# ocrickard/piper-swift

Hardware: AMD Instinct MI355X
Metric: audio-sec/wall-sec (RTF^-1) with ms/utterance, Piper VITS en_GB-medium geometry, scale-bench factor (higher is better)
Workload: dtype f32; 1 GPU; medium factor=8: 112 ids, 336 frames, 86016 samples (3.901 s audio) per utterance, 1 utterance per step per GPU; factor=8, phoneme_count=112, frames=336, samples=86016, parallelism=utterance-replicas x1 (one-shot RCCL weight broadcast)

## Files before the change

### piper-swift_amd/csrc/conv_win.h

```cpp
#pragma once
#include "common.h"

namespace ph {

struct ConvWinArgs {
  const float* x = nullptr;
  const float* x2 = nullptr;
  const float* x3 = nullptr;
  const float* w4 = nullptr;
  const float* bias = nullptr;
  const float* res = nullptr;
  const float* mrf_a = nullptr;
  const float* mrf_b = nullptr;
  float* y = nullptr;
  float pro_alpha = 1.0f;
  float out_alpha = 1.0f;
  int N = 1, Cin = 0, Cout = 0, K = 1, dil = 1, padL = 0;
  int Lin = 0;
  int Lout = 0;
  int y_len = 0;
  int ct_stride = 0, ct_pad = 0;
  const int* len_ptr = nullptr;
  int len_mul = 1;
};

size_t packed_conv_win_floats(int Cout, int Cin, int K);
size_t packed_convt_win_floats(int Cin, int Cout, int K, int stride);
int pack_conv_weights_win(hipStream_t s, const float* w, int Cout, int Cin, int K, float* packed);
int pack_convt_weights_win(hipStream_t s, const float* w, int Cin, int Cout, int K, int stride, int pad, float* packed);

bool conv_win_eligible(int Cout, int Cin, int K, int dil, int padL, int Lin, int Lout);
bool convt_win_eligible(int Cin, int Cout, int K, int stride, int pad, int Lin);

int launch_conv_win(piper_hip_ctx* ctx, hipStream_t s, const ConvWinArgs& a);
constexpr int kWinMulti = 3;
int launch_conv_win_multi(piper_hip_ctx* ctx, hipStream_t s, const ConvWinArgs* convs, int count);

size_t packed_conv_pipe_floats(int Cout, int Cin, int K);
size_t packed_convt_pipe_floats(int Cin, int Cout, int K, int stride);
int pack_conv_weights_pipe(hipStream_t s, const float* w, int Cout, int Cin, int K, float* packed);
int pack_convt_weights_pipe(hipStream_t s, const float* w, int Cin, int Cout, int K, int stride, int pad, float* packed);
bool conv_pipe_eligible(int Cout, int Cin, int K, int dil, int padL, int Lin, int Lout);
bool convt_pipe_eligible(int Cin, int Cout, int K, int stride, int pad, int Lin);
int launch_conv_pipe_multi(piper_hip_ctx* ctx, hipStream_t s, const ConvWinArgs* convs, int count);

struct RbPairArgs {
  const float* x = nullptr;
  float* y = nullptr;
  const float *wa4 = nullptr, *ba = nullptr, *wb4 = nullptr, *bb = nullptr;
  int Ka = 1, dila = 1, Kb = 1, dilb = 1;
  int res_a = 1, res_b_x = 0;
  float alpha = 0.1f;
  int N = 1, C = 0, L = 0;
  const int* len_ptr = nullptr;
  int len_mul = 1;
};
bool rb_pair_eligible(int C, int Ka, int dila, int Kb, int dilb, int L);
int launch_rb_pair_multi(piper_hip_ctx* ctx, hipStream_t s, const RbPairArgs* pairs, int count);

}
```

### piper-swift_amd/csrc/rb_pair.hip

```cpp
#include <algorithm>
#include <type_traits>

#include "conv_win.h"

namespace ph {
namespace {

typedef float f32x16 __attribute__((ext_vector_type(16)));

constexpr int kRA = 8;
constexpr int kStepPad = 16;
constexpr int kWN = 4, kNTW = 2, kT1 = kWN * kNTW;
constexpr int kColsA = 32 * kT1;
__host__ __device__ constexpr int halo_of(int pb) { return pb <= 16 ? 16 : 48; }
constexpr int kMaxReachB = 48;
constexpr int kStageU = 10;

struct RbPairMulti {
  RbPairArgs c[kWinMulti];
};

#ifdef PH_PAIR_TRACE
__device__ unsigned long long* ph_pair_trace_buf;
#define PH_STAMP(k) do { if (lane == 0 && round < 4 && ph_pair_trace_buf && blockIdx.x < 512) ph_pair_trace_buf[(((size_t)blockIdx.x * (MT * kWN) + wave) * 4 + round) * 8 + (k)] = __builtin_amdgcn_s_memtime(); } while (0)
#else
#define PH_STAMP(k) do { } while (0)
#endif

__device__ __forceinline__ float lrelu_max(float v, float alpha) { return fmaxf(v, v * alpha); }

__device__ __forceinline__ float bload(__amdgpu_buffer_rsrc_t r, int voff, int soff) {
  return __builtin_bit_cast(float, __builtin_amdgcn_raw_buffer_load_b32(r, voff, soff, 0));
}
__device__ __forceinline__ void bstore(__amdgpu_buffer_rsrc_t r, float v, int voff, int soff) {
  __builtin_amdgcn_raw_buffer_store_b32(__builtin_bit_cast(int, v), r, voff, soff, 0);
}

struct PairSched {
  int ntx[kWinMulti];
  int cnt[kWinMulti];
  int total, batch, order;
};

template <int MT>
__global__ __launch_bounds__(MT * kWN * 64, 2) void rb_pair_kernel(const RbPairMulti multi, const PairSched sch, const int Wx, const int W1,
                                                               const unsigned inv_w4) {
  extern __shared__ __attribute__((aligned(16))) float lds[];
  constexpr int BT = MT * kWN * 64;
  const int lane = threadIdx.x & 63;
  const int wave = __builtin_amdgcn_readfirstlane((int)(threadIdx.x >> 6));
  const int wm = wave % MT, wn = wave / MT;
  const int r = lane & 31, h = lane >> 5;
  constexpr int C = 32 * MT, C2 = C >> 1;
  float* xs = lds;
  float* x1s = lds + C * Wx + 4;
  float* biasS = x1s + C * W1;
  for (int i = threadIdx.x; i < kWinMulti * 2 * C; i += BT) {
    const int z = i / (2 * C), rem = i - z * 2 * C;
    const RbPairArgs& p = multi.c[(sch.order >> (4 * z)) & 15];
    biasS[i] = rem < C ? p.ba[rem] : p.bb[rem - C];
  }
  const int rowlane = wm * 32 + 4 * h;
  const unsigned lane16 = (unsigned)lane * 16u;
  const int G = (int)gridDim.x, bid = (int)blockIdx.x;

  struct Tile {
    const float *x, *wa4, *wb4;
    float* y;
    int bias_off;
    int Ka, dila, Kb, dilb, res_a, res_b_x, L, Lv, pa, pb, halo, c0, ga, shift, Sa, Spa, Sb, Spb, ntb;
    float alpha;
  };
  auto tile_index = [&](int round) {
    const int idx = round * G + ((round & 1) ? G - 1 - bid : bid);
    return idx < sch.total ? idx : -1;
  };
  auto setup = [&](int idx) {
    int z = 0, rem = idx;
    if (rem >= sch.cnt[0]) { rem -= sch.cnt[0]; z = 1; }
    if (z == 1 && rem >= sch.cnt[1]) { rem -= sch.cnt[1]; z = 2; }
    const RbPairArgs& p = multi.c[(sch.order >> (4 * z)) & 15];
    const int ntx = sch.ntx[z];
    const int n = __builtin_amdgcn_readfirstlane(rem / ntx);
    const int bx = rem - n * ntx;
    Tile t;
    t.x = p.x + (int64_t)n * C * p.L;
    t.y = p.y + (int64_t)n * C * p.L;
    t.wa4 = p.wa4; t.wb4 = p.wb4; t.bias_off = z * 2 * C;
    t.Ka = p.Ka; t.dila = p.dila; t.Kb = p.Kb; t.dilb = p.dilb; t.res_a = p.res_a; t.res_b_x = p.res_b_x; t.L = p.L; t.alpha = p.alpha;
    t.Lv = p.len_ptr ? min(p.len_ptr[n] * p.len_mul, p.L) : p.L;
    t.pa = (p.Ka - 1) * p.dila / 2; t.pb = (p.Kb - 1) * p.dilb / 2;
    t.halo = halo_of(t.pb);
    const int ncb = kColsA - 2 * t.halo;
    t.c0 = bx * ncb;
    const int g0 = t.c0 - t.halo - t.pa;
    t.ga = g0 & ~3;
    t.shift = g0 - t.ga;
    t.Sa = p.Ka * C2; t.Spa = (t.Sa + kStepPad - 1) / kStepPad * kStepPad;
    t.Sb = p.Kb * C2; t.Spb = (t.Sb + kStepPad - 1) / kStepPad * kStepPad;
    t.ntb = min(max((ncb >> 5) - wn * kNTW, 0), kNTW);
    return t;
  };

  float4 a[kRA];
  const char* wa = nullptr;
  auto load_a = [&](int slot, int ahead) { a[slot] = *(const float4*)(wa + ahead * 1024 + lane16); };
  auto ring_start = [&](const float* w4, int Sp) {
    wa = (const char*)w4 + (int64_t)wm * Sp * 256;
#pragma unroll
    for (int d = 0; d < kRA - 1; d++) load_a(d, d);
  };

  float4 pre[kStageU];
  const int W4 = Wx >> 2, total4 = C * W4;
  auto stage_issue = [&](const Tile& t, const int tx) {
#pragma unroll
    for (int u = 0; u < kStageU; u++) {
      const int ic = min(tx + u * BT, total4 - 1);
      const int row = (int)__umulhi((unsigned)ic, inv_w4);
      const int pos = t.ga + 4 * (ic - row * W4);
      pre[u] = *(const float4*)(t.x + (int64_t)row * t.L + ((pos >= 0 && pos < t.L) ? pos : 0));
    }
  };
  auto stage_commit = [&](const Tile& t, const int tx) {
#pragma unroll
    for (int u = 0; u < kStageU; u++) {
      const int i = tx + u * BT;
      const int ic = min(i, total4 - 1);
      const int row = (int)__umulhi((unsigned)ic, inv_w4);
      const int i4 = ic - row * W4;
      const int pos = t.ga + 4 * i4;
      const int nv = (pos >= 0 && pos < t.L) ? t.Lv - pos : 0;
      float4 v = pre[u];
      v.x = nv > 0 ? lrelu_max(v.x, t.alpha) : 0.0f; v.y = nv > 1 ? lrelu_max(v.y, t.alpha) : 0.0f;
      v.z = nv > 2 ? lrelu_max(v.z, t.alpha) : 0.0f; v.w = nv > 3 ? lrelu_max(v.w, t.alpha) : 0.0f;
      *(float4*)(xs + (i < total4 ? row * Wx + 4 * i4 : C * Wx)) = v;
    }
  };

  f32x16 acc[kNTW];
  auto run_conv = [&](auto nt_tag, const float* img, const int Wrow, const int S, const int Sp, const int dil, const int col0, const int bias_off) {
    constexpr int NT = decltype(nt_tag)::value;
#pragma unroll
    for (int g4 = 0; g4 < 4; g4++) {
      const float4 bv = *(const float4*)(biasS + bias_off + rowlane + 8 * g4);
#pragma unroll
      for (int j = 0; j < kNTW; j++) { acc[j][4 * g4] = bv.x; acc[j][4 * g4 + 1] = bv.y; acc[j][4 * g4 + 2] = bv.z; acc[j][4 * g4 + 3] = bv.w; }
    }
    const int lbase = h * Wrow + col0 + r;
    int sidx = 0, c_n = 0, left = S - 1;
    const int wrap_delta = dil - 2 * Wrow * (C2 - 1);
    float b[2][NT][4];
    auto read_b4 = [&](int slot) {
#pragma unroll
      for (int e = 0; e < 4; e++) {
#pragma unroll
        for (int j = 0; j < NT; j++) b[slot][j][e] = img[lbase + sidx + 32 * j];
        c_n++;
        const bool wrap = c_n == C2;
        c_n = wrap ? 0 : c_n;
        const int delta = wrap ? wrap_delta : 2 * Wrow;
        sidx += left > 0 ? delta : 0;
        left--;
      }
    };
    auto group = [&](int u) {
      load_a((u + kRA - 1) % kRA, kRA - 1 + u);
      read_b4((u + 1) & 1);
      __builtin_amdgcn_sched_barrier(0);
      const float av[4] = {a[u].x, a[u].y, a[u].z, a[u].w};
#pragma unroll
      for (int e = 0; e < 4; e++)
#pragma unroll
        for (int j = 0; j < NT; j++) acc[j] = __builtin_amdgcn_mfma_f32_32x32x2f32(av[e], b[u & 1][j][e], acc[j], 0, 0, 0);
    };
    read_b4(0);
    const int Gr = Sp >> 2, full = Gr / kRA;
    if (full > 0) {
#pragma unroll
      for (int u = 0; u < kRA; u++) group(u);
      wa += kRA * 1024;
    }
    for (int g = 1; g < full; g++) {
#pragma unroll
      for (int u = 0; u < kRA; u++) group(u);
      wa += kRA * 1024;
    }
    const int rem = Gr - full * kRA;
#pragma unroll
    for (int u = 0; u < kRA - 1; u++)
      if (u < rem) group(u);
  };

  Tile cur = setup(tile_index(0));
  ring_start(cur.wa4, cur.Spa);
  stage_issue(cur, (int)threadIdx.x);
  stage_commit(cur, (int)threadIdx.x);
  __syncthreads();

  for (int round = 0;; round++) {
    const int nidx = tile_index(round + 1);
    const bool has_next = nidx >= 0;
    const Tile nxt = has_next ? setup(nidx) : cur;
    int tx = (int)threadIdx.x, rl = rowlane, rr = r;
    asm volatile("" : "+v"(tx), "+v"(rl), "+v"(rr));
    float resx[kNTW][16];
    auto load_res = [&](int gres0) {
      const __amdgpu_buffer_rsrc_t rx = __builtin_amdgcn_make_buffer_rsrc((void*)cur.x, 0, C * cur.L * 4, 0x00020000);
#pragma unroll
      for (int j = 0; j < kNTW; j++) {
        const int g = gres0 + (wn * kNTW + j) * 32 + rr;
        const int voff = (g >= 0 && g < cur.L) ? (rl * cur.L + g) * 4 : -4;
#pragma unroll
        for (int q = 0; q < 16; q++) resx[j][q] = bload(rx, voff, ((q & 3) + 8 * (q >> 2)) * cur.L * 4);
      }
    };

    PH_STAMP(0);
    __builtin_amdgcn_s_waitcnt(0x0F70);
    PH_STAMP(1);
    if (has_next) stage_issue(nxt, tx);

    const bool live = cur.c0 < cur.Lv;
    if (live) run_conv(std::integral_constant<int, kNTW>{}, xs, Wx, cur.Sa, cur.Spa, cur.dila, cur.shift + wn * kNTW * 32, cur.bias_off);
    PH_STAMP(2);
    if (live) ring_start(cur.wb4, cur.Spb);
    if (live && cur.res_a) load_res(cur.c0 - cur.halo);
    __syncthreads();
    PH_STAMP(3);

    if (live) {
#pragma unroll
      for (int j = 0; j < kNTW; j++) {
        const int colw = (wn * kNTW + j) * 32 + rr;
        const int g = cur.c0 - cur.halo + colw;
        const bool in = g >= 0 && g < cur.Lv;
#pragma unroll
        for (int q = 0; q < 16; q++) {
          const int rq = (q & 3) + 8 * (q >> 2);
          const int o = (rl + rq) * W1 + colw;
          float v = acc[j][q];
          if (cur.res_a) v += resx[j][q];
          v = in ? v : 0.0f;
          x1s[o] = lrelu_max(v, cur.alpha);
          if (!cur.res_b_x) xs[o] = v;
        }
      }
    }
    __syncthreads();

    PH_STAMP(4);
    if (live && cur.ntb > 0) {
      const int col0b = cur.halo - cur.pb + wn * kNTW * 32;
      __builtin_amdgcn_s_waitcnt(0x0F70);
      if (cur.ntb == 2) run_conv(std::integral_constant<int, 2>{}, x1s, W1, cur.Sb, cur.Spb, cur.dilb, col0b, cur.bias_off + C);
      else run_conv(std::integral_constant<int, 1>{}, x1s, W1, cur.Sb, cur.Spb, cur.dilb, col0b, cur.bias_off + C);
    }
    PH_STAMP(5);
    if (has_next) ring_start(nxt.wa4, nxt.Spa);
    if (live && cur.res_b_x && cur.ntb > 0) load_res(cur.c0);
    if (live && cur.ntb > 0) {
      const __amdgpu_buffer_rsrc_t ry = __builtin_amdgcn_make_buffer_rsrc((void*)cur.y, 0, C * cur.L * 4, 0x00020000);
#pragma unroll
      for (int j = 0; j < kNTW; j++) {
        if (j >= cur.ntb) break;
        const int colo = (wn * kNTW + j) * 32 + rr;
        const int g = cur.c0 + colo;
        const int voff = g < cur.L ? (rl * cur.L + g) * 4 : -4;
#pragma unroll
        for (int q = 0; q < 16; q++) {
          const int rq = (q & 3) + 8 * (q >> 2);
          float v = acc[j][q];
          v += cur.res_b_x ? resx[j][q] : xs[(rl + rq) * W1 + cur.halo + colo];
          bstore(ry, v, voff, rq * cur.L * 4);
        }
      }
    }
    PH_STAMP(6);
    if (!has_next) break;
    __syncthreads();
    stage_commit(nxt, tx);
    __syncthreads();
    PH_STAMP(7);
    cur = nxt;
  }
}

struct PairGeom {
  int Wx, W1;
  size_t lds;
};

PairGeom pair_geom(int C, int pa_max, int pb_max) {
  auto pad = [](int w, bool odd32) {
    w = (w + 3) & ~3;
    if (odd32) while ((w & 63) != 32) w += 4;
    return w;
  };
  PairGeom g;
  for (int pass = 0; pass < 2; pass++) {
    g.Wx = pad(kColsA + 2 * pa_max + 3, pass == 0);
    g.W1 = pad(kColsA, pass == 0);
    (void)pb_max;
    g.lds = ((size_t)C * g.Wx + 4 + (size_t)C * g.W1 + (size_t)kWinMulti * 2 * C) * sizeof(float);
    if (g.lds <= 160 * 1024 && (C * g.Wx) / 4 <= kStageU * (C / 32) * kWN * 64) break;
  }
  return g;
}

template <int MT>
void launch_pair_inst(piper_hip_ctx* ctx, hipStream_t s, const RbPairMulti& m, const PairSched& sch, const PairGeom& g) {
  static bool raised[kMaxDevices] = {};
  if (g.lds > 64 * 1024 && lds_optin_needed(raised))
    (void)hipFuncSetAttribute((const void*)rb_pair_kernel<MT>, hipFuncAttributeMaxDynamicSharedMemorySize, 160 * 1024);
  const unsigned inv = (unsigned)(0x100000000ull / (unsigned)(g.Wx >> 2)) + 1u;
  const int per_cu = std::max(1, std::min(2, (int)((size_t)160 * 1024 / g.lds)));
  const int grid = std::min(sch.total, per_cu * ctx->num_cus);
  hipLaunchKernelGGL((rb_pair_kernel<MT>), dim3(grid), dim3(MT * kWN * 64), g.lds, s, m, sch, g.Wx, g.W1, inv);
}

}

#ifdef PH_PAIR_TRACE
void rb_pair_set_trace(unsigned long long* buf) { (void)hipMemcpyToSymbol(HIP_SYMBOL(ph_pair_trace_buf), &buf, sizeof buf); }
#endif

bool rb_pair_eligible(int C, int Ka, int dila, int Kb, int dilb, int L) {
  if (C != 32 && C != 64) return false;
  if (Ka < 1 || Kb < 1 || !(Ka & 1) || !(Kb & 1) || dila < 1 || dilb < 1) return false;
  if (L < 4 || (L & 3)) return false;
  const int pa = (Ka - 1) * dila / 2, pb = (Kb - 1) * dilb / 2;
  if (pb > kMaxReachB) return false;
  if ((int64_t)C * (kColsA + 2 * pa + 70) >= (1 << 20)) return false;
  const PairGeom g = pair_geom(C, pa, pb);
  return g.lds <= 160 * 1024 && (C * g.Wx) / 4 <= kStageU * (C / 32) * kWN * 64;
}

int launch_rb_pair_multi(piper_hip_ctx* ctx, hipStream_t s, const RbPairArgs* pairs, int count) {
  if (count < 1 || count > kWinMulti) PH_FAIL(PIPER_HIP_ERR_ARG, "rb_pair: %d pairs in one launch (1..%d)", count, kWinMulti);
  const RbPairArgs& a = pairs[0];
  if (a.N <= 0 || a.L <= 0) return PIPER_HIP_OK;
  int pa_max = 0, pb_max = 0;
  int idx[kWinMulti] = {0, 1, 2};
  for (int i = 0; i < count; i++) {
    const RbPairArgs& b = pairs[i];
    if (b.N != a.N || b.C != a.C || b.L != a.L) PH_FAIL(PIPER_HIP_ERR_SHAPE, "rb_pair: pairs of one launch must share N, C and L");
    if (!rb_pair_eligible(b.C, b.Ka, b.dila, b.Kb, b.dilb, b.L)) PH_FAIL(PIPER_HIP_ERR_UNSUPPORTED, "rb_pair: geometry not covered (C=%d K=%d,%d d=%d,%d L=%d)", b.C, b.Ka, b.Kb, b.dila, b.dilb, b.L);
    if (!(b.alpha > 0.0f && b.alpha < 1.0f)) PH_FAIL(PIPER_HIP_ERR_UNSUPPORTED, "rb_pair: LeakyReLU slope %g outside (0,1)", (double)b.alpha);
    if (!b.x || !b.y || !b.wa4 || !b.wb4 || !b.ba || !b.bb) PH_FAIL(PIPER_HIP_ERR_ARG, "rb_pair: null operand");
    pa_max = std::max(pa_max, (b.Ka - 1) * b.dila / 2);
    pb_max = std::max(pb_max, (b.Kb - 1) * b.dilb / 2);
  }
  const PairGeom g = pair_geom(a.C, pa_max, pb_max);
  if (g.lds > 160 * 1024 || (a.C * g.Wx) / 4 > kStageU * (a.C / 32) * kWN * 64)
    PH_FAIL(PIPER_HIP_ERR_UNSUPPORTED, "rb_pair: window of %zu bytes (row %d) exceeds LDS / the staging registers", g.lds, g.Wx);
  std::sort(idx, idx + count, [&](int l, int r2) { return pairs[l].Ka + pairs[l].Kb > pairs[r2].Ka + pairs[r2].Kb; });
  PairSched sch = {};
  sch.batch = a.N;
  for (int i = 0; i < count; i++) {
    const RbPairArgs& b = pairs[idx[i]];
    sch.order |= idx[i] << (4 * i);
    sch.ntx[i] = (int)ceil_div(a.L, kColsA - 2 * halo_of((b.Kb - 1) * b.dilb / 2));
    sch.cnt[i] = sch.ntx[i] * a.N;
    sch.total += sch.cnt[i];
  }
  for (int i = count; i < kWinMulti; i++) { sch.ntx[i] = 1; sch.cnt[i] = 0; }
  RbPairMulti m;
  for (int i = 0; i < kWinMulti; i++) m.c[i] = pairs[i < count ? i : 0];
  if (a.C == 32) launch_pair_inst<1>(ctx, s, m, sch, g);
  else launch_pair_inst<2>(ctx, s, m, sch, g);
  hipError_t e = hipGetLastError();
  if (e != hipSuccess) PH_FAIL(PIPER_HIP_ERR_LAUNCH, "rb_pair launch failed: %s", hipGetErrorString(e));
  return PIPER_HIP_OK;
}

}
namespace ph { namespace { PH_WARM(rb_pair, (rb_pair_kernel<1>)); } }
```

Before: 5373 audio-sec/wall-sec.

## Add streaming rb_pair kernel that walks columns with a rolling halo window

```diff
diff --git a/piper-swift_amd/csrc/conv_win.h b/piper-swift_amd/csrc/conv_win.h
--- a/piper-swift_amd/csrc/conv_win.h
+++ b/piper-swift_amd/csrc/conv_win.h
@@ -57,5 +57,6 @@
 };
 bool rb_pair_eligible(int C, int Ka, int dila, int Kb, int dilb, int L);
 int launch_rb_pair_multi(piper_hip_ctx* ctx, hipStream_t s, const RbPairArgs* pairs, int count);
+bool launch_rb_pair_stream(piper_hip_ctx* ctx, hipStream_t s, const RbPairArgs* pairs, int count);
 
 }
diff --git a/piper-swift_amd/csrc/rb_pair.hip b/piper-swift_amd/csrc/rb_pair.hip
--- a/piper-swift_amd/csrc/rb_pair.hip
+++ b/piper-swift_amd/csrc/rb_pair.hip
@@ -1,40 +1,20 @@
 #include <algorithm>
 #include <type_traits>
 
-#include "conv_win.h"
+#include "rb_pair_common.h"
 
 namespace ph {
 namespace {
 
-typedef float f32x16 __attribute__((ext_vector_type(16)));
-
-constexpr int kRA = 8;
-constexpr int kStepPad = 16;
-constexpr int kWN = 4, kNTW = 2, kT1 = kWN * kNTW;
 constexpr int kColsA = 32 * kT1;
 __host__ __device__ constexpr int halo_of(int pb) { return pb <= 16 ? 16 : 48; }
 constexpr int kMaxReachB = 48;
-constexpr int kStageU = 10;
-
-struct RbPairMulti {
-  RbPairArgs c[kWinMulti];
-};
-
 #ifdef PH_PAIR_TRACE
 __device__ unsigned long long* ph_pair_trace_buf;
 #define PH_STAMP(k) do { if (lane == 0 && round < 4 && ph_pair_trace_buf && blockIdx.x < 512) ph_pair_trace_buf[(((size_t)blockIdx.x * (MT * kWN) + wave) * 4 + round) * 8 + (k)] = __builtin_amdgcn_s_memtime(); } while (0)
 #else
 #define PH_STAMP(k) do { } while (0)
 #endif
-
-__device__ __forceinline__ float lrelu_max(float v, float alpha) { return fmaxf(v, v * alpha); }
-
-__device__ __forceinline__ float bload(__amdgpu_buffer_rsrc_t r, int voff, int soff) {
-  return __builtin_bit_cast(float, __builtin_amdgcn_raw_buffer_load_b32(r, voff, soff, 0));
-}
-__device__ __forceinline__ void bstore(__amdgpu_buffer_rsrc_t r, float v, int voff, int soff) {
-  __builtin_amdgcn_raw_buffer_store_b32(__builtin_bit_cast(int, v), r, voff, soff, 0);
-}
 
 struct PairSched {
   int ntx[kWinMulti];
@@ -102,94 +82,17 @@
     return t;
   };
 
-  float4 a[kRA];
-  const char* wa = nullptr;
-  auto load_a = [&](int slot, int ahead) { a[slot] = *(const float4*)(wa + ahead * 1024 + lane16); };
-  auto ring_start = [&](const float* w4, int Sp) {
-    wa = (const char*)w4 + (int64_t)wm * Sp * 256;
-#pragma unroll
-    for (int d = 0; d < kRA - 1; d++) load_a(d, d);
-  };
+  PairRing ring;
+  auto ring_start = [&](const float* w4, int Sp) { ring.start(w4, Sp, wm, lane16); };
 
   float4 pre[kStageU];
   const int W4 = Wx >> 2, total4 = C * W4;
-  auto stage_issue = [&](const Tile& t, const int tx) {
-#pragma unroll
-    for (int u = 0; u < kStageU; u++) {
-      const int ic = min(tx + u * BT, total4 - 1);
-      const int row = (int)__umulhi((unsigned)ic, inv_w4);
-      const int pos = t.ga + 4 * (ic - row * W4);
-      pre[u] = *(const float4*)(t.x + (int64_t)row * t.L + ((pos >= 0 && pos < t.L) ? pos : 0));
-    }
-  };
-  auto stage_commit = [&](const Tile& t, const int tx) {
-#pragma unroll
-    for (int u = 0; u < kStageU; u++) {
-      const int i = tx + u * BT;
-      const int ic = min(i, total4 - 1);
-      const int row = (int)__umulhi((unsigned)ic, inv_w4);
-      const int i4 = ic - row * W4;
-      const int pos = t.ga + 4 * i4;
-      const int nv = (pos >= 0 && pos < t.L) ? t.Lv - pos : 0;
-      float4 v = pre[u];
-      v.x = nv > 0 ? lrelu_max(v.x, t.alpha) : 0.0f; v.y = nv > 1 ? lrelu_max(v.y, t.alpha) : 0.0f;
-      v.z = nv > 2 ? lrelu_max(v.z, t.alpha) : 0.0f; v.w = nv > 3 ? lrelu_max(v.w, t.alpha) : 0.0f;
-      *(float4*)(xs + (i < total4 ? row * Wx + 4 * i4 : C * Wx)) = v;
-    }
-  };
+  auto stage_issue = [&](const Tile& t, const int tx) { pair_stage_issue<BT>(pre, t.x, t.L, t.ga, tx, W4, total4, inv_w4); };
+  auto stage_commit = [&](const Tile& t, const int tx) { pair_stage_commit<BT>(pre, xs, Wx, C, t.L, t.Lv, t.ga, t.alpha, tx, W4, total4, inv_w4); };
 
   f32x16 acc[kNTW];
   auto run_conv = [&](auto nt_tag, const float* img, const int Wrow, const int S, const int Sp, const int dil, const int col0, const int bias_off) {
-    constexpr int NT = decltype(nt_tag)::value;
-#pragma unroll
-    for (int g4 = 0; g4 < 4; g4++) {
-      const float4 bv = *(const float4*)(biasS + bias_off + rowlane + 8 * g4);
-#pragma unroll
-      for (int j = 0; j < kNTW; j++) { acc[j][4 * g4] = bv.x; acc[j][4 * g4 + 1] = bv.y; acc[j][4 * g4 + 2] = bv.z; acc[j][4 * g4 + 3] = bv.w; }
-    }
-    const int lbase = h * Wrow + col0 + r;
-    int sidx = 0, c_n = 0, left = S - 1;
-    const int wrap_delta = dil - 2 * Wrow * (C2 - 1);
-    float b[2][NT][4];
-    auto read_b4 = [&](int slot) {
-#pragma unroll
-      for (int e = 0; e < 4; e++) {
-#pragma unroll
-        for (int j = 0; j < NT; j++) b[slot][j][e] = img[lbase + sidx + 32 * j];
-        c_n++;
-        const bool wrap = c_n == C2;
-        c_n = wrap ? 0 : c_n;
-        const int delta = wrap ? wrap_delta : 2 * Wrow;
-        sidx += left > 0 ? delta : 0;
-        left--;
-      }
-    };
-    auto group = [&](int u) {
-      load_a((u + kRA - 1) % kRA, kRA - 1 + u);
-      read_b4((u + 1) & 1);
-      __builtin_amdgcn_sched_barrier(0);
-      const float av[4] = {a[u].x, a[u].y, a[u].z, a[u].w};
-#pragma unroll
-      for (int e = 0; e < 4; e++)
-#pragma unroll
-        for (int j = 0; j < NT; j++) acc[j] = __builtin_amdgcn_mfma_f32_32x32x2f32(av[e], b[u & 1][j][e], acc[j], 0, 0, 0);
-    };
-    read_b4(0);
-    const int Gr = Sp >> 2, full = Gr / kRA;
-    if (full > 0) {
-#pragma unroll
-      for (int u = 0; u < kRA; u++) group(u);
-      wa += kRA * 1024;
-    }
-    for (int g = 1; g < full; g++) {
-#pragma unroll
-      for (int u = 0; u < kRA; u++) group(u);
-      wa += kRA * 1024;
-    }
-    const int rem = Gr - full * kRA;
-#pragma unroll
-    for (int u = 0; u < kRA - 1; u++)
-      if (u < rem) group(u);
+    pair_run_conv<C, decltype(nt_tag)::value, kNTW>(acc, ring, lane16, biasS, rowlane, h, r, img, Wrow, S, Sp, dil, col0, bias_off);
   };
 
   Tile cur = setup(tile_index(0));
@@ -351,6 +254,12 @@
     pa_max = std::max(pa_max, (b.Ka - 1) * b.dila / 2);
     pb_max = std::max(pb_max, (b.Kb - 1) * b.dilb / 2);
   }
+  static const bool stream_off = [] { const char* e = getenv("PIPER_HIP_RB_STREAM"); return e && e[0] == '0'; }();
+  if (!stream_off && launch_rb_pair_stream(ctx, s, pairs, count)) {
+    hipError_t e = hipGetLastError();
+    if (e != hipSuccess) PH_FAIL(PIPER_HIP_ERR_LAUNCH, "rb_pair_stream launch failed: %s", hipGetErrorString(e));
+    return PIPER_HIP_OK;
+  }
   const PairGeom g = pair_geom(a.C, pa_max, pb_max);
   if (g.lds > 160 * 1024 || (a.C * g.Wx) / 4 > kStageU * (a.C / 32) * kWN * 64)
     PH_FAIL(PIPER_HIP_ERR_UNSUPPORTED, "rb_pair: window of %zu bytes (row %d) exceeds LDS / the staging registers", g.lds, g.Wx);
diff --git a/piper-swift_amd/csrc/rb_pair_common.h b/piper-swift_amd/csrc/rb_pair_common.h
--- /dev/null
+++ b/piper-swift_amd/csrc/rb_pair_common.h
@@ -0,0 +1,126 @@
+#pragma once
+
+#include "conv_win.h"
+
+namespace ph {
+namespace {
+
+typedef float f32x16 __attribute__((ext_vector_type(16)));
+
+constexpr int kRA = 8;
+constexpr int kStepPad = 16;
+constexpr int kWN = 4, kNTW = 2, kT1 = kWN * kNTW;
+constexpr int kStageU = 10;
+
+struct RbPairMulti {
+  RbPairArgs c[kWinMulti];
+};
+
+__device__ __forceinline__ float lrelu_max(float v, float alpha) { return fmaxf(v, v * alpha); }
+
+__device__ __forceinline__ float bload(__amdgpu_buffer_rsrc_t r, int voff, int soff) {
+  return __builtin_bit_cast(float, __builtin_amdgcn_raw_buffer_load_b32(r, voff, soff, 0));
+}
+__device__ __forceinline__ void bstore(__amdgpu_buffer_rsrc_t r, float v, int voff, int soff) {
+  __builtin_amdgcn_raw_buffer_store_b32(__builtin_bit_cast(int, v), r, voff, soff, 0);
+}
+
+struct PairRing {
+  float4 a[kRA];
+  const char* wa;
+  __device__ __forceinline__ void load(int slot, int ahead, unsigned lane16) { a[slot] = *(const float4*)(wa + ahead * 1024 + lane16); }
+  __device__ __forceinline__ void start(const float* w4, int Sp, int wm, unsigned lane16) {
+    wa = (const char*)w4 + (int64_t)wm * Sp * 256;
+#pragma unroll
+    for (int d = 0; d < kRA - 1; d++) load(d, d, lane16);
+  }
+};
+
+template <int BT>
+__device__ __forceinline__ void pair_stage_issue(float4 (&pre)[kStageU], const float* x, const int L, const int ga, const int tx, const int W4,
+                                                 const int total4, const unsigned inv_w4) {
+#pragma unroll
+  for (int u = 0; u < kStageU; u++) {
+    const int ic = min(tx + u * BT, total4 - 1);
+    const int row = (int)__umulhi((unsigned)ic, inv_w4);
+    const int pos = ga + 4 * (ic - row * W4);
+    pre[u] = *(const float4*)(x + (int64_t)row * L + ((pos >= 0 && pos < L) ? pos : 0));
+  }
+}
+template <int BT>
+__device__ __forceinline__ void pair_stage_commit(const float4 (&pre)[kStageU], float* xs, const int Wx, const int C, const int L, const int Lv,
+                                                  const int ga, const float alpha, const int tx, const int W4, const int total4,
+                                                  const unsigned inv_w4) {
+#pragma unroll
+  for (int u = 0; u < kStageU; u++) {
+    const int i = tx + u * BT;
+    const int ic = min(i, total4 - 1);
+    const int row = (int)__umulhi((unsigned)ic, inv_w4);
+    const int i4 = ic - row * W4;
+    const int pos = ga + 4 * i4;
+    const int nv = (pos >= 0 && pos < L) ? Lv - pos : 0;
+    float4 v = pre[u];
+    v.x = nv > 0 ? lrelu_max(v.x, alpha) : 0.0f; v.y = nv > 1 ? lrelu_max(v.y, alpha) : 0.0f;
+    v.z = nv > 2 ? lrelu_max(v.z, alpha) : 0.0f; v.w = nv > 3 ? lrelu_max(v.w, alpha) : 0.0f;
+    *(float4*)(xs + (i < total4 ? row * Wx + 4 * i4 : C * Wx)) = v;
+  }
+}
+
+template <int C, int NT, int NA>
+__device__ __forceinline__ void pair_run_conv(f32x16 (&acc)[NA], PairRing& ring, const unsigned lane16, const float* biasS, const int rowlane,
+                                              const int h, const int r, const float* img, const int Wrow, const int S, const int Sp,
+                                              const int dil, const int col0, const int bias_off) {
+  constexpr int C2 = C >> 1;
+#pragma unroll
+  for (int g4 = 0; g4 < 4; g4++) {
+    const float4 bv = *(const float4*)(biasS + bias_off + rowlane + 8 * g4);
+#pragma unroll
+    for (int j = 0; j < NA; j++) { acc[j][4 * g4] = bv.x; acc[j][4 * g4 + 1] = bv.y; acc[j][4 * g4 + 2] = bv.z; acc[j][4 * g4 + 3] = bv.w; }
+  }
+  const int lbase = h * Wrow + col0 + r;
+  int sidx = 0, c_n = 0, left = S - 1;
+  const int wrap_delta = dil - 2 * Wrow * (C2 - 1);
+  float b[2][NT][4];
+  auto read_b4 = [&](int slot) {
+#pragma unroll
+    for (int e = 0; e < 4; e++) {
+#pragma unroll
+      for (int j = 0; j < NT; j++) b[slot][j][e] = img[lbase + sidx + 32 * j];
+      c_n++;
+      const bool wrap = c_n == C2;
+      c_n = wrap ? 0 : c_n;
+      const int delta = wrap ? wrap_delta : 2 * Wrow;
+      sidx += left > 0 ? delta : 0;
+      left--;
+    }
+  };
+  auto group = [&](int u) {
+    ring.load((u + kRA - 1) % kRA, kRA - 1 + u, lane16);
+    read_b4((u + 1) & 1);
+    __builtin_amdgcn_sched_barrier(0);
+    const float av[4] = {ring.a[u].x, ring.a[u].y, ring.a[u].z, ring.a[u].w};
+#pragma unroll
+    for (int e = 0; e < 4; e++)
+#pragma unroll
+      for (int j = 0; j < NT; j++) acc[j] = __builtin_amdgcn_mfma_f32_32x32x2f32(av[e], b[u & 1][j][e], acc[j], 0, 0, 0);
+  };
+  read_b4(0);
+  const int Gr = Sp >> 2, full = Gr / kRA;
+  if (full > 0) {
+#pragma unroll
+    for (int u = 0; u < kRA; u++) group(u);
+    ring.wa += kRA * 1024;
+  }
+  for (int g = 1; g < full; g++) {
+#pragma unroll
+    for (int u = 0; u < kRA; u++) group(u);
+    ring.wa += kRA * 1024;
+  }
+  const int rem = Gr - full * kRA;
+#pragma unroll
+  for (int u = 0; u < kRA - 1; u++)
+    if (u < rem) group(u);
+}
+
+}
+}
diff --git a/piper-swift_amd/csrc/rb_pair_stream.hip b/piper-swift_amd/csrc/rb_pair_stream.hip
--- /dev/null
+++ b/piper-swift_amd/csrc/rb_pair_stream.hip
@@ -0,0 +1,264 @@
+#include <algorithm>
+
+#include "rb_pair_common.h"
+
+namespace ph {
+namespace {
+
+constexpr int kSS = 32 * kWN;
+constexpr int kMaxReachB = 48;
+
+#ifdef PH_PAIR_TRACE
+__device__ unsigned long long* ph_pair_stream_trace_buf;
+#define PH_SSTAMP(k) do { if (lane == 0 && step < 8 && ph_pair_stream_trace_buf && blockIdx.x < 512) ph_pair_stream_trace_buf[(((size_t)blockIdx.x * (MT * kWN) + wave) * 8 + step) * 8 + (k)] = __builtin_amdgcn_s_memtime(); } while (0)
+#else
+#define PH_SSTAMP(k) do { } while (0)
+#endif
+
+struct StreamSched {
+  int first[kWinMulti + 1];
+  int per_item[kWinMulti];
+  int base[kWinMulti], extra[kWinMulti];
+  int order;
+};
+
+template <int MT>
+__global__ __launch_bounds__(MT * kWN * 64, 2) void rb_pair_stream_kernel(const RbPairMulti multi, const StreamSched sch, const int Wx,
+                                                                      const int W1, const int has_raw, const unsigned inv_w4) {
+  extern __shared__ __attribute__((aligned(16))) float lds[];
+  constexpr int BT = MT * kWN * 64;
+  constexpr int C = 32 * MT, C2 = C >> 1;
+  const int lane = threadIdx.x & 63;
+  const int wave = __builtin_amdgcn_readfirstlane((int)(threadIdx.x >> 6));
+  const int wm = wave % MT, wn = wave / MT;
+  const int r = lane & 31, h = lane >> 5;
+  const int bid = (int)blockIdx.x;
+
+  int z = 0;
+  if (bid >= sch.first[1]) z = 1;
+  if (bid >= sch.first[2]) z = 2;
+  int k = bid - sch.first[z], n = 0;
+  while (k >= sch.per_item[z]) { k -= sch.per_item[z]; n++; }
+  const RbPairArgs& p = multi.c[(sch.order >> (4 * z)) & 15];
+  const int L = p.L;
+  const int Lv = p.len_ptr ? min(p.len_ptr[n] * p.len_mul, L) : L;
+  const int pa = (p.Ka - 1) * p.dila / 2, pb = (p.Kb - 1) * p.dilb / 2;
+  const int ncb = 256 - 2 * (pb <= 16 ? 16 : 48);
+  const int lim = min(L, (Lv + ncb - 1) / ncb * ncb);
+  const int t0 = k * sch.base[z] + min(k, sch.extra[z]);
+  const int a = 32 * t0;
+  const int b = min(min(a + 32 * (sch.base[z] + (k < sch.extra[z] ? 1 : 0)), L), lim);
+  if (a >= b) return;
+  const int nsteps = (b - a + kSS - 1) / kSS;
+  const int Q = 2 * pb;
+  const float* x = p.x + (int64_t)n * C * L;
+  float* y = p.y + (int64_t)n * C * L;
+  const float alpha = p.alpha;
+  const int Sa = p.Ka * C2, Spa = (Sa + kStepPad - 1) / kStepPad * kStepPad;
+  const int Sb = p.Kb * C2, Spb = (Sb + kStepPad - 1) / kStepPad * kStepPad;
+
+  float* xs = lds;
+  float* x1s = lds + C * Wx + 4;
+  float* raws = x1s + C * W1;
+  float* biasS = raws + (has_raw ? C * W1 : 0);
+  for (int i = threadIdx.x; i < 2 * C; i += BT) biasS[i] = i < C ? p.ba[i] : p.bb[i - C];
+
+  const int rowlane = wm * 32 + 4 * h;
+  const unsigned lane16 = (unsigned)lane * 16u;
+  PairRing ring;
+  float4 pre[kStageU];
+  const int W4 = Wx >> 2, total4 = C * W4;
+  f32x16 acc[1];
+  float resx[16];
+
+  auto front = [&](int s) { return a + pb + (s - 1) * kSS; };
+  auto need_a = [&](int s) { return s == 0 ? 32 * wn + 32 > kSS - Q : (s - 1) * kSS + 32 * wn < b - a; };
+  auto stage_ga = [&](int s) { return (front(s) - pa) & ~3; };
+  auto load_res = [&](int g0) {
+    const __amdgpu_buffer_rsrc_t rx = __builtin_amdgcn_make_buffer_rsrc((void*)x, 0, C * L * 4, 0x00020000);
+    const int g = g0 + r;
+    const int voff = (g >= 0 && g < L) ? (rowlane * L + g) * 4 : -4;
+#pragma unroll
+    for (int q = 0; q < 16; q++) resx[q] = bload(rx, voff, ((q & 3) + 8 * (q >> 2)) * L * 4);
+  };
+
+  if (need_a(0)) ring.start(p.wa4, Spa, wm, lane16);
+  pair_stage_issue<BT>(pre, x, L, stage_ga(0), (int)threadIdx.x, W4, total4, inv_w4);
+  pair_stage_commit<BT>(pre, xs, Wx, C, L, Lv, stage_ga(0), alpha, (int)threadIdx.x, W4, total4, inv_w4);
+  __syncthreads();
+
+  for (int step = 0; step <= nsteps; step++) {
+    const bool has_next = step < nsteps;
+    const int e = front(step);
+    const int shift = (e - pa) - stage_ga(step);
+    const bool na = need_a(step);
+    const int ob = a + (step - 1) * kSS + 32 * wn;
+    const bool nb = step > 0 && ob < b;
+    PH_SSTAMP(0);
+    __builtin_amdgcn_s_waitcnt(0x0F70);
+    PH_SSTAMP(1);
+    if (has_next) pair_stage_issue<BT>(pre, x, L, stage_ga(step + 1), (int)threadIdx.x, W4, total4, inv_w4);
+
+    if (na) pair_run_conv<C, 1, 1>(acc, ring, lane16, biasS, rowlane, h, r, xs, Wx, Sa, Spa, p.dila, shift + 32 * wn, 0);
+    PH_SSTAMP(2);
+    if (nb) ring.start(p.wb4, Spb, wm, lane16);
+    if (na && p.res_a) load_res(e + 32 * wn);
+    __syncthreads();
+    PH_SSTAMP(3);
+    if (na) {
+      const int g = e + 32 * wn + r;
+      const bool in = g >= 0 && g < Lv;
+#pragma unroll
+      for (int q = 0; q < 16; q++) {
+        const int o = (rowlane + (q & 3) + 8 * (q >> 2)) * W1 + Q + 32 * wn + r;
+        float v = acc[0][q];
+        if (p.res_a) v += resx[q];
+        v = in ? v : 0.0f;
+        x1s[o] = lrelu_max(v, alpha);
+        if (!p.res_b_x) raws[o] = v;
+      }
+    }
+    __syncthreads();
+    PH_SSTAMP(4);
+
+    if (nb) {
+      __builtin_amdgcn_s_waitcnt(0x0F70);
+      pair_run_conv<C, 1, 1>(acc, ring, lane16, biasS, rowlane, h, r, x1s, W1, Sb, Spb, p.dilb, 32 * wn, C);
+    }
+    PH_SSTAMP(5);
+    if (has_next && need_a(step + 1)) ring.start(p.wa4, Spa, wm, lane16);
+    if (nb && p.res_b_x) load_res(ob);
+    if (nb) {
+      const __amdgpu_buffer_rsrc_t ry = __builtin_amdgcn_make_buffer_rsrc((void*)y, 0, C * L * 4, 0x00020000);
+      const int g = ob + r;
+      const int voff = g < L ? (rowlane * L + g) * 4 : -4;
+#pragma unroll
+      for (int q = 0; q < 16; q++) {
+        const int rq = (q & 3) + 8 * (q >> 2);
+        float v = acc[0][q];
+        v += p.res_b_x ? resx[q] : raws[(rowlane + rq) * W1 + pb + 32 * wn + r];
+        bstore(ry, v, voff, rq * L * 4);
+      }
+    }
+    PH_SSTAMP(6);
+    if (!has_next) break;
+    __syncthreads();
+    pair_stage_commit<BT>(pre, xs, Wx, C, L, Lv, stage_ga(step + 1), alpha, (int)threadIdx.x, W4, total4, inv_w4);
+    {
+      const int nq = (Q + 3) >> 2;
+      for (int i = threadIdx.x; i < C * 32; i += BT) {
+        const int row = i >> 5, c4 = i & 31;
+        if (c4 < nq) {
+          float* src = x1s + row * W1 + kSS + 4 * c4;
+          *(float4*)(src - kSS) = *(const float4*)src;
+          if (has_raw) *(float4*)(src - kSS + C * W1) = *(const float4*)(src + C * W1);
+        }
+      }
+    }
+    __syncthreads();
+    PH_SSTAMP(7);
+  }
+}
+
+struct StreamGeom {
+  int Wx, W1, has_raw;
+  size_t lds;
+};
+StreamGeom stream_geom(int C, int pa_max, int pb_max, int has_raw) {
+  auto pad = [](int w, bool odd32) {
+    w = (w + 3) & ~3;
+    if (odd32) while ((w & 63) != 32) w += 4;
+    return w;
+  };
+  const size_t budget = C == 32 ? 80 * 1024 : 160 * 1024;
+  StreamGeom g;
+  g.has_raw = has_raw;
+  for (int pass = 0; pass < 2; pass++) {
+    g.Wx = pad(kSS + 2 * pa_max + 3, pass == 0);
+    g.W1 = pad(kSS + 2 * pb_max + 3, pass == 0);
+    g.lds = ((size_t)C * g.Wx + 4 + (size_t)C * g.W1 * (1 + has_raw) + 2 * (size_t)C) * sizeof(float);
+    if (g.lds <= budget) break;
+  }
+  return g;
+}
+
+double stream_block_cost(int C, int Ka, int Kb, int cols) {
+  constexpr double kFixed = 4.0;
+  double t = Ka + kFixed;
+  for (int c = cols; c > 0; c -= kSS) {
+    const int tiles = std::min(kSS, c) / 32 + (c % 32 && c < kSS ? 1 : 0);
+    t += (C == 64 && tiles <= 2 ? 0.5 : 1.0) * (Ka + Kb) + kFixed;
+  }
+  return t;
+}
+
+template <int MT>
+void launch_stream_inst(piper_hip_ctx* ctx, hipStream_t s, const RbPairMulti& m, const StreamSched& sch, const StreamGeom& g, int grid) {
+  static bool raised[kMaxDevices] = {};
+  if (g.lds > 64 * 1024 && lds_optin_needed(raised))
+    (void)hipFuncSetAttribute((const void*)rb_pair_stream_kernel<MT>, hipFuncAttributeMaxDynamicSharedMemorySize, 160 * 1024);
+  const unsigned inv = (unsigned)(0x100000000ull / (unsigned)(g.Wx >> 2)) + 1u;
+  hipLaunchKernelGGL((rb_pair_stream_kernel<MT>), dim3(grid), dim3(MT * kWN * 64), g.lds, s, m, sch, g.Wx, g.W1, g.has_raw, inv);
+}
+
+}
+
+#ifdef PH_PAIR_TRACE
+void rb_pair_stream_set_trace(unsigned long long* buf) { (void)hipMemcpyToSymbol(HIP_SYMBOL(ph_pair_stream_trace_buf), &buf, sizeof buf); }
+#endif
+
+bool launch_rb_pair_stream(piper_hip_ctx* ctx, hipStream_t s, const RbPairArgs* pairs, int count) {
+  const RbPairArgs& a0 = pairs[0];
+  const int C = a0.C, N = a0.N, L = a0.L;
+  int pa_max = 0, pb_max = 0, has_raw = 0;
+  for (int i = 0; i < count; i++) {
+    pa_max = std::max(pa_max, (pairs[i].Ka - 1) * pairs[i].dila / 2);
+    pb_max = std::max(pb_max, (pairs[i].Kb - 1) * pairs[i].dilb / 2);
+    has_raw |= pairs[i].res_b_x ? 0 : 1;
+    if (pairs[i].res_b_x) return false;
+  }
+  if (C != 32) return false;
+  if (!has_raw || pb_max > kMaxReachB || 2 * pb_max > kSS) return false;
+  const StreamGeom g = stream_geom(C, pa_max, pb_max, has_raw);
+  if (g.lds > (C == 32 ? 80u : 160u) * 1024 || (C * g.Wx) / 4 > kStageU * (C / 32) * kWN * 64) return false;
+  if ((int64_t)C * g.Wx >= (1 << 20)) return false;
+
+  const int per_cu = C == 32 ? 2 : 1;
+  const int G = per_cu * ctx->num_cus;
+  const int tiles = (L + 31) / 32;
+  int idx[kWinMulti] = {0, 1, 2};
+  std::sort(idx, idx + count, [&](int l, int r2) { return pairs[l].Ka + pairs[l].Kb > pairs[r2].Ka + pairs[r2].Kb; });
+  int B[kWinMulti] = {1, 1, 1};
+  auto cost = [&](int i) {
+    const RbPairArgs& p = pairs[idx[i]];
+    return stream_block_cost(C, p.Ka, p.Kb, std::min(L, 32 * ((tiles + B[i] - 1) / B[i])));
+  };
+  int used = count * N;
+  while (used + N <= G) {
+    int worst = -1;
+    double wc = 0.0;
+    for (int i = 0; i < count; i++)
+      if (B[i] < tiles && cost(i) > wc) { wc = cost(i); worst = i; }
+    if (worst < 0) break;
+    B[worst]++;
+    used += N;
+  }
+  StreamSched sch = {};
+  sch.first[0] = 0;
+  for (int i = 0; i < count; i++) {
+    sch.order |= idx[i] << (4 * i);
+    sch.per_item[i] = B[i];
+    sch.base[i] = tiles / B[i];
+    sch.extra[i] = tiles % B[i];
+    sch.first[i + 1] = sch.first[i] + B[i] * N;
+  }
+  for (int i = count; i < kWinMulti; i++) { sch.per_item[i] = 1; sch.first[i + 1] = sch.first[i]; }
+  RbPairMulti m;
+  for (int i = 0; i < kWinMulti; i++) m.c[i] = pairs[i < count ? i : 0];
+  if (C == 32) launch_stream_inst<1>(ctx, s, m, sch, g, used);
+  else launch_stream_inst<2>(ctx, s, m, sch, g, used);
+  return true;
+}
+
+}
+namespace ph { namespace { PH_WARM(rb_pair_stream, (rb_pair_stream_kernel<1>)); } }
```

New measurement: 5394 audio-sec/wall-sec (median of 6 runs). Within noise of the previous version (+0.4%).
